# zeyadmohamedabdo/Visual-Question-Answering-VQA-system

Measured on AMD Instinct MI355X. Metric: image-question pairs/sec (train step), higher is better.
Workload: dtype bf16; 1 GPU; VQA train step fwd+CE+bwd+allreduce+clip+AdamW, batch 512/GPU, 3x224x224 images, 20 tokens, d=256, 4 text layers, 49 image tokens, 1000 answers, dropout on (BASELINE configs[2]); batch_per_gpu=512, global_batch=512, parallelism=dp1, reducer=off

## Files before the change

include/vqa_hip.h:

```cpp
#ifndef VQA_HIP_H
#define VQA_HIP_H
#include <stdint.h>
#ifdef __cplusplus
extern "C" {
#endif
typedef struct ihipStream_t* hipStream_t;

int vqa_igemm_mtiles(int M, int N, int loader);
int vqa_igemm_variant(int dtype, int loader, int M, int N, int Kw, int B, int H, int W, int C, int Ho, int Wo,
                      int R, int S, int stride, int pad);
int vqa_igemm(int dtype, int loader, const void* a, const void* w, void* out, const float* bias, const void* addend,
              const void* addmask, const void* outmask , float* stats, int M, int N, int Kw, int B, int H, int W, int C, int Ho, int Wo,
              int R, int S, int stride, int pad, int transposed, int relu, float drop_p, unsigned long long drop_seed,
              int stats_mode ,
              hipStream_t stream);
int vqa_linear_dgrad_act(int dtype, const void* dz, const void* wt, void* dx, const void* addend, const void* outact, float drop_p,
                         int M, int Kin, int N, hipStream_t stream);
int vqa_wgrad_plan(int dtype, int loader, int M, int N, int Kw, int B, int H, int W, int C, int R, int S, long long* ws_floats,
                   int* kind, int* tile_n, int* tile_k, int* nsplit);
int vqa_wgrad(int dtype, int loader, const void* dy, const void* x, float* dw, int M, int N, int Kw, int B, int H, int W,
              int C, int Ho, int Wo, int R, int S, int stride, int pad, float* ws, long long ws_floats, hipStream_t stream);
int vqa_pack_rows(int dtype, const float* in, void* out, int N, int K, int Kp, hipStream_t stream);
int vqa_pack_transpose(int dtype, const float* in, void* out, int N, int T, int C, int ldo, int col0, int flip, hipStream_t stream);
int vqa_pack_transpose_batch(int dtype, const float* flat, void* out, const long long* desc, int nd, int total_blocks, hipStream_t stream);
int vqa_fold_bn_batch(int dtype, const float* flat, void* wout, float* bout, const long long* desc, int nd, int total_blocks, float eps, hipStream_t stream);
int vqa_mx_quant(int dtype, const void* in, uint8_t* q, uint8_t* s, int M, int C, hipStream_t stream);
int vqa_fold_bn_mxfp8(const float* flat, uint8_t* wq, uint8_t* ws, float* bout, const long long* desc, int nd, int total_blocks, float eps,
                      hipStream_t stream);
int vqa_conv_mxfp8(const uint8_t* a, const uint8_t* as, const uint8_t* w, const uint8_t* ws, const float* bias, const void* addend,
                   void* out, uint8_t* oq, uint8_t* os, int M, int N, int B, int H, int W, int C, int Ho, int Wo, int R, int S,
                   int stride, int pad, int relu, hipStream_t stream);
int vqa_conv3x3_c64p_blocks(int B, int H, int W);
int vqa_conv3x3_c64p_bnred(const void* x, const void* w, void* out, const void* bn_y, const float* bn_coef, unsigned long long* bn_facc,
                           int B, int H, int W, hipStream_t stream);
int vqa_conv3x3_c64p_epi(const void* x, const void* w, void* out, const void* addend, const void* addmask, const void* outmask,
                         int B, int H, int W, hipStream_t stream);
int vqa_conv3x3_c64p(const void* x, const void* w, void* out, float* stats, int B, int H, int W,
                     int stats_mode , hipStream_t stream);
int vqa_gemm8p(const void* A, const void* B, void* C, int M, int N, int K, hipStream_t stream);
int vqa_gemm4w(const void* A, const void* B, void* C, int M, int N, int K, hipStream_t stream);
int vqa_conv8p_ok(int B, int H, int W, int C, int N);
int vqa_conv8p(const void* x, const void* w, void* out, unsigned long long* stats,
               const void* addend, const void* addmask, const void* outmask ,
               const void* bn_y, const float* bn_coef, unsigned long long* bn_facc ,
               int bn_selfmask ,
               const void* bn_y2, const float* bn_coef2 ,
               int B, int H, int W, int C, int N, int transposed, int stride , hipStream_t stream);
int vqa_conv3x3_c64p_bn(const void* y, const unsigned long long* acc, const float* gamma, const float* beta, float* running_mean,
                        float* running_var, long long* num_batches_tracked, float* coef_out, const void* w, void* out, float* stats,
                        int B, int H, int W, int stats_mode, double count, float momentum, float eps, hipStream_t stream);
int vqa_wgrad3x3_c64_bn_ok(int B, int H, int W);
int vqa_wgrad3x3_c64_bn(const void* y, const float* coef, const void* dy, float* dw , int B, int H, int W,
                        float* ws , long long ws_floats, hipStream_t stream);
int vqa_wgrad3x3_c128_blocks(int B, int H, int W);
int vqa_wgrad3x3_c128(const void* x, const void* dy, float* dw, int B, int H, int W, float* ws, long long ws_floats, hipStream_t stream);
int vqa_wgrad3x3_c64_blocks(int B, int H, int W);
int vqa_wgrad3x3_c64(const void* x, const void* dy, float* dw , int B, int H, int W,
                     float* ws ,
                     long long ws_floats, hipStream_t stream);
long long vqa_wgrad_group_ws(int dtype, int njobs, const int* M, const int* N, const int* Kw);
int vqa_wgrad_group(int dtype, int njobs, const void* const* dy, const void* const* x, float* const* dw, const int* M, const int* N,
                    const int* Kw, float* ws, long long ws_floats, hipStream_t stream);
int vqa_slab_reduce(const float* ws, float* dw, int nslabs, long long n, hipStream_t stream);
int vqa_dgrad_s2(int dtype, const void* dy, const void* dyd, const void* wt, void* out, int B, int H, int W, int C,
                 int Ho, int Wo, int N, int R, int pad, hipStream_t stream);
int vqa_stem_conv_blocks(int B, int H, int W);
int vqa_stem_pack(const float* w_krsc, void* wstem, hipStream_t stream);
int vqa_stem_conv(const float* img, const void* wstem, void* out, float* stats, int B, int H, int W, hipStream_t stream);
int vqa_stem_conv_pool_ok(int B, int H, int W);
int vqa_stem_conv_pool(const float* img, const void* wstem, const float* coef, void* out, int B, int H, int W, hipStream_t stream);
int vqa_stem_wgrad_blocks(int B, int H, int W);
int vqa_stem_wgrad(const float* img, const void* dy, float* dw , int B, int H, int W,
                   float* ws , long long ws_floats, hipStream_t stream);
int vqa_stem_wgrad_fused(const float* img, const void* y, const void* dpool, const uint8_t* idx, const float* coef,
                         const float* bcoef, float* dw, int B, int H, int W, float* ws, long long ws_floats, hipStream_t stream);
int vqa_stem_dgrad_pack(int dtype, const float* w_krsc, void* wpk, hipStream_t stream);
int vqa_stem_dgrad(int dtype, const void* dy, const void* wpk, float* dimg, int B, int H, int W, hipStream_t stream);
int vqa_stem_dgrad_fused_ok(int B, int H, int W);
int vqa_stem_dgrad_fused(const void* y, const void* dpool, const uint8_t* idx, const float* coef, const float* bcoef, const void* wpk,
                         float* dimg, int B, int H, int W, hipStream_t stream);

int vqa_bn_stats_finalize(const float* part, int tiles, int C, double count, const float* gamma, const float* beta,
                          float* running_mean, float* running_var, long long* num_batches_tracked, float momentum, float eps,
                          double* scratch , float* coef, hipStream_t stream);
int vqa_bn_eval_coef(int C, const float* gamma, const float* beta, const float* running_mean, const float* running_var,
                     float eps, float* coef, hipStream_t stream);
int vqa_bn_apply(int dtype, const void* y, const float* coef, const void* res, const float* rcoef, void* out,
                 long long numel, int C, int relu, hipStream_t stream);
int vqa_bn_apply_pool_chunks(int dtype, int HW, int C);
int vqa_bn_apply_pool(int dtype, const void* y, const float* coef, const void* res, const float* rcoef, void* out, int B, int HW, int C,
                      int relu, float* part, hipStream_t stream);
int vqa_bn_acc_words(int K, int C);
int vqa_bn_apply_acc(int dtype, const void* y, const unsigned long long* acc, const float* gamma, const float* beta, float* running_mean,
                     float* running_var, long long* num_batches_tracked, float* coef_out, const void* res,
                     const unsigned long long* racc, const float* rgamma, const float* rbeta, float* rrunning_mean, float* rrunning_var,
                     long long* rnum_batches_tracked, float* rcoef_out, void* out, int B, int HW, int C, int relu, double count,
                     float momentum, float eps, float* pool_part, hipStream_t stream);
int vqa_bn_bwd_blocks(long long rows);
int vqa_bn_bwd_reduce(int dtype, const void* dout, const void* outact, const void* y, const float* coef, const void* y2,
                      const float* coef2, float* slab , long long rows,
                      int C, int self_mask , int acc_mode, hipStream_t stream);
int vqa_bn_bwd_apply_acc(int dtype, const void* dout, const void* outact, const void* y, const unsigned long long* facc, const float* gamma,
                         const float* coef, float* dgamma, float* dbeta, void* dy, const void* y2, const float* gamma2, const float* coef2,
                         float* dgamma2, float* dbeta2, void* dy2, long long numel, int C, double count, int self_mask, hipStream_t stream);
int vqa_bn_bwd_finalize(const float* slab, int nblk, int C, int which, double count, const float* gamma, const float* coef,
                        int training, float* dgamma, float* dbeta, float* bcoef , hipStream_t stream);
int vqa_bn_bwd_apply(int dtype, const void* dout, const void* outact, const void* y, const float* bcoef, void* dy,
                     const void* y2, const float* bcoef2, void* dy2, long long numel, int C, const float* mask_coef ,
                     hipStream_t stream);

int vqa_stem_pool_fwd(int dtype, const void* y, const float* coef, void* out, uint8_t* idx, int B, int H, int W, int C, hipStream_t stream);
int vqa_stem_bwd_apply(int dtype, const void* dpool, const uint8_t* idx, const void* y, const float* coef, const float* bcoef,
                       void* dy, int B, int H, int W, int C, hipStream_t stream);

int vqa_se_fwd(int dtype, const void* x, const float* w1, const float* w2, float* pooled, float* hidden, float* scale,
               void* out, int B, int HW, int C, int Cr,
               const float* pool_part , int pool_chunks , hipStream_t stream);
int vqa_se_bwd_blocks(int dtype, int B, int HW, int C);
// ... 123 lines not shown
```

visual-question-answering-vqa-system_amd/_lib.py:

```python
from __future__ import annotations

import ctypes as C
import os

import torch

_HERE = os.path.dirname(os.path.abspath(__file__))
LIB_PATH = os.path.join(_HERE, "libvqa_hip.so")

P, I, F, D, LL, ULL = C.c_void_p, C.c_int, C.c_float, C.c_double, C.c_longlong, C.c_ulonglong

SIGNATURES = {
    "vqa_gemm8p": [P, P, P, I, I, I, P],
    "vqa_gemm4w": [P, P, P, I, I, I, P],
    "vqa_conv8p_ok": [I, I, I, I, I],
    "vqa_conv8p": [P, P, P, P, P, P, P, P, P, P, I, P, P, I, I, I, I, I, I, I, P],
    "vqa_igemm_mtiles": [I, I, I],
    "vqa_igemm_variant": [I] * 15,
    "vqa_igemm": [I, I, P, P, P, P, P, P, P, P] + [I] * 15 + [F, ULL, I, P],
    "vqa_linear_dgrad_act": [I, P, P, P, P, P, F, I, I, I, P],
    "vqa_wgrad_plan": [I] * 11 + [P, P, P, P, P],
    "vqa_wgrad": [I, I, P, P, P] + [I] * 13 + [P, LL, P],
    "vqa_pack_rows": [I, P, P, I, I, I, P],
    "vqa_pack_transpose": [I, P, P, I, I, I, I, I, I, P],
    "vqa_pack_transpose_batch": [I, P, P, P, I, I, P],
    "vqa_fold_bn_batch": [I, P, P, P, P, I, I, F, P],
    "vqa_mx_quant": [I, P, P, P, I, I, P],
    "vqa_fold_bn_mxfp8": [P, P, P, P, P, I, I, F, P],
    "vqa_conv_mxfp8": [P] * 9 + [I] * 13 + [P],
    "vqa_conv3x3_c64p_blocks": [I, I, I],
    "vqa_conv3x3_c64p": [P, P, P, P, I, I, I, I, P],
    "vqa_conv3x3_c64p_epi": [P, P, P, P, P, P, I, I, I, P],
    "vqa_conv3x3_c64p_bnred": [P, P, P, P, P, P, I, I, I, P],
    "vqa_conv3x3_c64p_bn": [P, P, P, P, P, P, P, P, P, P, P, I, I, I, I, D, F, F, P],
    "vqa_wgrad3x3_c64_bn_ok": [I, I, I],
    "vqa_wgrad3x3_c64_bn": [P, P, P, P, I, I, I, P, LL, P],
    "vqa_wgrad3x3_c128_blocks": [I, I, I],
    "vqa_wgrad3x3_c128": [P, P, P, I, I, I, P, LL, P],
    "vqa_wgrad3x3_c64_blocks": [I, I, I],
    "vqa_wgrad3x3_c64": [P, P, P, I, I, I, P, LL, P],
    "vqa_wgrad_group_ws": [I, I, P, P, P],
    "vqa_wgrad_group": [I, I, P, P, P, P, P, P, P, LL, P],
    "vqa_slab_reduce": [P, P, I, LL, P],
    "vqa_dgrad_s2": [I, P, P, P, P, I, I, I, I, I, I, I, I, I, P],
    "vqa_stem_conv_blocks": [I, I, I],
    "vqa_stem_pack": [P, P, P],
    "vqa_stem_conv": [P, P, P, P, I, I, I, P],
    "vqa_stem_conv_pool_ok": [I, I, I],
    "vqa_stem_conv_pool": [P, P, P, P, I, I, I, P],
    "vqa_stem_wgrad_blocks": [I, I, I],
    "vqa_stem_wgrad": [P, P, P, I, I, I, P, LL, P],
    "vqa_stem_wgrad_fused": [P, P, P, P, P, P, P, I, I, I, P, LL, P],
    "vqa_stem_dgrad_pack": [I, P, P, P],
    "vqa_stem_dgrad": [I, P, P, P, I, I, I, P],
    "vqa_stem_dgrad_fused_ok": [I, I, I],
    "vqa_stem_dgrad_fused": [P, P, P, P, P, P, P, I, I, I, P],
    "vqa_bn_stats_finalize": [P, I, I, D, P, P, P, P, P, F, F, P, P, P],
    "vqa_bn_eval_coef": [I, P, P, P, P, F, P, P],
    "vqa_bn_apply": [I, P, P, P, P, P, LL, I, I, P],
    "vqa_bn_apply_pool_chunks": [I, I, I],
    "vqa_bn_apply_pool": [I, P, P, P, P, P, I, I, I, I, P, P],
    "vqa_se_bwd_blocks": [I, I, I, I],
    "vqa_se_bwd_scratch": [I, I, I, I, I],
    "vqa_bn_bwd_blocks": [LL],
    "vqa_bn_bwd_reduce": [I, P, P, P, P, P, P, P, LL, I, I, I, P],
    "vqa_bn_acc_words": [I, I],
    "vqa_bn_apply_acc": [I, P, P, P, P, P, P, P, P, P, P, P, P, P, P, P, P, P, I, I, I, I, D, F, F, P, P],
    "vqa_bn_bwd_apply_acc": [I, P, P, P, P, P, P, P, P, P, P, P, P, P, P, P, LL, I, D, I, P],
    "vqa_bn_bwd_finalize": [P, I, I, I, D, P, P, I, P, P, P, P],
    "vqa_bn_bwd_apply": [I, P, P, P, P, P, P, P, P, LL, I, P, P],
    "vqa_stem_pool_fwd": [I, P, P, P, P, I, I, I, I, P],
    "vqa_stem_bwd_apply": [I, P, P, P, P, P, P, I, I, I, I, P],
    "vqa_se_fwd": [I, P, P, P, P, P, P, P, I, I, I, I, P, I, P],
    "vqa_se_bwd": [I, P, P, P, P, P, P, P, P, P, P, P, I, I, I, I, I, P, P, P, I, P],
    "vqa_spatial_fwd": [I, P, P, P, P, P, P, I, I, I, I, P],
    "vqa_spatial_bwd_scratch": [I, I, I],
    "vqa_spatial_bwd": [I, P, P, P, P, P, P, P, P, P, I, I, I, I, P],
    "vqa_nhwc_to_nchw": [I, P, P, I, I, I, P],
    "vqa_nchw_to_nhwc": [I, P, P, I, I, I, P],
    "vqa_embed_fwd": [I, P, P, P, P, I, I, I, I, F, F, ULL, P],
    "vqa_embed_bwd": [I, P, P, P, I, I, I, F, F, ULL, P],
    "vqa_layernorm_fwd": [I, P, P, P, P, P, I, I, F, F, ULL, P, I, P],
    "vqa_layernorm_bwd_ws": [I, I, I, I],
    "vqa_layernorm_bwd": [I, P, P, P, P, P, P, P, P, I, I, F, ULL, P, I, P, I, P],
    "vqa_layernorm_bwd_folds": [I, I, I, I, P],
    "vqa_attention_fwd": [I, P, P, P, I, I, I, P, P, P, I, I, I, I, I, I, F, ULL, P],
    "vqa_attention_fwd_mfma": [P, P, P, I, I, I, P, P, P, I, I, I, I, I, I, F, ULL, P],
    "vqa_attention_fwd_idx": [I, P, P, P, I, I, I, P, I, P, P, P, I, I, I, I, I, I, P],
    "vqa_attention_fwd_mfma_idx": [P, P, P, I, I, I, P, I, P, P, P, I, I, I, I, I, I, P],
    "vqa_attention_bwd": [I, P, I, P, P, P, I, I, I, P, P, P, P, I, I, I, I, I, I, I, I, F, ULL, P],
    "vqa_accuracy_update": [P, P, P, I, I, P],
    "vqa_attention_bwd_mfma": [P, I, P, P, P, I, I, I, P, P, P, P, I, I, I, I, I, I, I, I, F, ULL, P],
    "vqa_attention_bwd_dp": [I, P, I, P, P, P, I, I, I, P, P, P, P, P, I, I, I, I, I, I, I, I, F, ULL, P],
    "vqa_attention_bwd_mfma_dp": [P, I, P, P, P, I, I, I, P, P, P, P, P, I, I, I, I, I, I, I, I, F, ULL, P],
    "vqa_index_csr": [P, I, I, P, P, P],
    "vqa_attention_fwd_idx_train": [I, P, P, P, I, I, I, P, I, P, P, P, I, I, I, I, I, I, F, ULL, P],
    "vqa_attention_fwd_mfma_idx_train": [P, P, P, I, I, I, P, I, P, P, P, I, I, I, I, I, I, F, ULL, P],
    "vqa_attention_bwd_idx": [I, P, I, P, P, P, I, I, I, P, P, P, I, P, P, P, I, I, I, I, I, I, I, I, F, ULL, P],
    "vqa_attention_bwd_mfma_idx": [P, I, P, P, P, I, I, I, P, P, P, I, P, P, P, I, I, I, I, I, I, I, I, F, ULL, P],
    "vqa_masked_pool_fwd": [I, P, P, P, I, I, I, I, I, P],
    "vqa_masked_pool_bwd": [I, P, I, I, P, P, P, I, I, I, P],
    "vqa_masked_pool_pair_fwd": [I, P, P, P, P, I, I, I, P],
    "vqa_masked_pool_pair_bwd": [I, P, P, P, P, I, I, I, P],
    "vqa_gate_fwd": [I, P, P, P, I, I, P],
    "vqa_gate_bwd": [I, P, P, P, P, P, I, I, P],
    "vqa_add": [I, P, P, P, LL, P],
    "vqa_grad_tap_add": [I, P, P, I, I, I, I, P],
    "vqa_bias_act_bwd_ws": [I, I, I],
    "vqa_bias_act_bwd": [I, P, P, P, P, I, I, F, ULL, P, I, P],
    "vqa_bias_act_bwd_fold_rows": [I, I, I],
    "vqa_fold_group": [I, P, P, P, P, P, P, P, P],
    "vqa_cross_entropy": [I, P, P, P, P, P, I, I, F, P, P, P],
    "vqa_answer_scores": [P, P, P, P, I, I, I, I, P, P],
    "vqa_cross_entropy_soft": [I, P, P, P, I, P, P, P, I, I, F, P, P, P, P, P],
    "vqa_challenge_accuracy_update": [P, P, P, I, P, I, I, P],
    "vqa_convert": [I, I, P, P, LL, P],
    "vqa_sumsq": [P, LL, P, P],
    "vqa_image_normalize": [P, P, P, I, I, I, F, F, F, F, F, F, P],
    "vqa_image_color_jitter": [P, P, P, I, I, I, P, P, F, F, F, F, F, F, P, P],
    "vqa_image_resize_ws": [I, P, P, I, I, I],
    "vqa_image_resize": [P, P, P, P, P, I, I, I, I, I, P, P, P, F, F, F, F, F, F, P, LL, P],
    "vqa_pack_tokens": [P, P, P, P, I, I, I, I, I, I, P],
    "vqa_adamw": [P, P, P, P, LL, F, F, F, F, F, LL, P, F, F, P, P, P, P],
    "vqa_sumsq_ranges": [P, P, I, LL, P, P],
    "vqa_adamw_ranges": [P, P, P, P, P, I, LL, F, F, F, F, F, LL, P, F, F, P, P, P, P, I, P, P],
}
_RET_LL = {"vqa_image_resize_ws", "vqa_wgrad_group_ws", "vqa_spatial_bwd_scratch", "vqa_se_bwd_scratch", "vqa_layernorm_bwd_ws", "vqa_bias_act_bwd_ws"}
_NO_STATUS = _RET_LL | {"vqa_wgrad3x3_c64_blocks", "vqa_bn_acc_words", "vqa_bn_apply_pool_chunks", "vqa_se_bwd_blocks", "vqa_wgrad3x3_c128_blocks", "vqa_layernorm_bwd_folds", "vqa_bias_act_bwd_fold_rows", "vqa_conv3x3_c64p_blocks", "vqa_stem_wgrad_blocks", "vqa_igemm_mtiles", "vqa_igemm_variant", "vqa_bn_bwd_blocks", "vqa_stem_conv_blocks", "vqa_stem_conv_pool_ok", "vqa_stem_dgrad_fused_ok", "vqa_wgrad3x3_c64_bn_ok", "vqa_conv8p_ok"}

_lib = None


def lib() -> C.CDLL:
    global _lib
    if _lib is None:
        if not os.path.exists(LIB_PATH):
            raise RuntimeError(f"{LIB_PATH} is missing: build it with __graft_entry__.build() "
                               "(hipcc --offload-arch=gfx950); there is no CPU fallback")
        L = C.CDLL(LIB_PATH)
        for name, args in SIGNATURES.items():
            fn = getattr(L, name)
            fn.argtypes = args
            fn.restype = LL if name in _RET_LL else I
        _lib = L
    return _lib


def ptr(t):
    return None if t is None else t.data_ptr()


def stream() -> int:
    return torch.cuda.current_stream().cuda_stream


_HOOK = [None]


def call(name: str, *args):
    fn = getattr(lib(), name)
    hook = _HOOK[0]
    done = hook(name, args) if hook is not None else None
    rc = fn(*args, stream())
    if done is not None:
        done()
    if rc != 0:
        raise RuntimeError(f"{name} failed with status {rc}" + (" (argument/shape error)" if rc == 1000 else " (hipError_t)"))


def count(name: str, *args) -> int:
    assert name in _NO_STATUS
    return getattr(lib(), name)(*args)


def dt(t_or_dtype) -> int:
    d = t_or_dtype.dtype if isinstance(t_or_dtype, torch.Tensor) else t_or_dtype
    if d == torch.float32:
        return 0
    if d == torch.bfloat16:
        return 1
    raise TypeError(f"unsupported dtype {d}")
# ... 1 lines not shown
```

visual-question-answering-vqa-system_amd/build.py:

```python
import os
import subprocess
import sys

HERE = os.path.dirname(os.path.abspath(__file__))
CSRC = os.path.join(HERE, "csrc")
SOURCES = ["gemm_conv.hip", "cnn_ops.hip", "token_ops.hip", "stem_conv.hip", "conv_c64.hip", "input_ops.hip", "gemm8p.hip", "mxfp8.hip", "stem_dgrad.hip"]
LIB = os.path.join(HERE, "libvqa_hip.so")
HIPCC = os.environ.get("HIPCC", "/opt/rocm/bin/hipcc")
FLAGS = ["--offload-arch=gfx950", "-O3", "-std=c++17", "-fPIC", "-Wno-unused-result"]


def _stale():
    if not os.path.exists(LIB):
        return True
    t = os.path.getmtime(LIB)
    import glob
    deps = [os.path.join(CSRC, f) for f in SOURCES] + glob.glob(os.path.join(CSRC, "*.h"))
    return any(os.path.getmtime(d) > t for d in deps)


def build_lib(force=False, verbose=True):
    if not force and not _stale():
        return LIB
    objs = []
    procs = []
    for src in SOURCES:
        obj = os.path.join(CSRC, src.replace(".hip", ".o"))
        objs.append(obj)
        cmd = [HIPCC] + FLAGS + ["-c", os.path.join(CSRC, src), "-o", obj]
        if verbose:
            print(" ".join(cmd), flush=True)
        procs.append((cmd, subprocess.Popen(cmd)))
    for cmd, p in procs:
        if p.wait() != 0:
            raise RuntimeError("hipcc failed: " + " ".join(cmd))
    cmd = [HIPCC, "--offload-arch=gfx950", "-shared", "-fPIC", "-o", LIB] + objs
    if verbose:
        print(" ".join(cmd), flush=True)
    subprocess.check_call(cmd)
    return LIB


if __name__ == "__main__":
    build_lib(force="--force" in sys.argv)
    print(LIB)
```

visual-question-answering-vqa-system_amd/engine.py:

```python
from __future__ import annotations

import math
from typing import Callable, Dict, List, Optional

import torch

from . import kernels as K
from . import layout as LY
from ._lib import call, dt, ptr


def _streams_overlap(a: "torch.cuda.Stream", b: "torch.cuda.Stream", cycles: int = 1_500_000) -> bool:
    ea, eb = torch.cuda.Event(), torch.cuda.Event()
    with torch.cuda.stream(a):
        torch.cuda._sleep(cycles)
        ea.record()
    with torch.cuda.stream(b):
        torch.cuda._sleep(1000)
        eb.record()
    eb.synchronize()
    ok = not ea.query()
    ea.synchronize()
    return ok

# ... 1 lines not shown
def pick_concurrent_streams(device, n: int, avoid=(), tries: int = 12):
    main = torch.cuda.current_stream(device)
    if torch.cuda.is_current_stream_capturing():
        return tuple(torch.cuda.Stream(device=device) for _ in range(n))
    chosen, spare = [], []
    for _ in range(tries):
        if len(chosen) == n:
            break
        c = torch.cuda.Stream(device=device)
        if all(_streams_overlap(o, c) for o in [main, *avoid, *chosen]):
            chosen.append(c)
        else:
            spare.append(c)
    while len(chosen) < n:
        chosen.append(spare.pop(0) if spare else torch.cuda.Stream(device=device))
    return tuple(chosen)


class HipEngine:
    def __init__(self, cfg: dict, entries: List[LY.Entry], flat: torch.Tensor, buffers: Dict[str, torch.Tensor],
                 compute_dtype: torch.dtype):
        self.cfg = cfg
        self.entries = entries
        self.E = {e.name: e for e in entries}
        self.flat = flat
        self.buf = buffers
        self.dtype = compute_dtype
        self.seed_base = 0x5EED
        self.seed_rank = None
        self.step_id = 0
        self.wsrc = flat
        self._wsrc_fresh = False
        self._wt: Dict[str, torch.Tensor] = {}
        self._wt_plan: Dict[str, tuple] = {}
        self._wt_table = None
        self._wt_buf = None
        self._deferred = []
        self._keep = []
        self._wgq = []
        self._foldq = []
        self._foldq2 = []
        self._plan = None
        self._bwd_G = None
        self.fuse_act_dgrad = True
        self.fuse_se_pool = True
        self.fuse_se_bnred = True
        self.fuse_bn_finalize = True
        self.fuse_bn_conv = True
        self.use_conv8p = True
        self.conv8p_n_multiple = 128
        self.conv8p_bwd_n_multiple = 128
        self.pack_off_main = True
        self.hoist_cross = True
        self.use_c64p_epi = True
        self.fuse_bn1_reduce = True
        self.use_conv8p_bwd = True
        self._accbuf = None
        self._accpos = 0
        self._stem_fcoef = None
        self.fold_eval = True
        self._fold = None
        self.infer_precision = "bf16"
        self._foldmx = None
        self.stem_w = None
        self.side, self.side2 = pick_concurrent_streams(flat.device, 2) if flat.is_cuda else (None, None)
        self.two_streams = True
        self.capture = None
        self.capture_io = None
        self.fuse_stem_eval = True
        self.mark = None

    def P(self, name):
        e = self.E[name]
        return self.flat[e.offset: e.offset + e.numel]

    def Wm(self, name):
        return LY.mat_of(self.wsrc, self.E[name])

    def _packT(self, key, pieces, rows, ld):
        t = self._wt.get(key)
        if t is None:
            t = torch.empty((rows, ld), device=self.flat.device, dtype=self.dtype)
            for off, n, tt, c, col0, flip in pieces:
                K.pack_transpose(self.flat[off: off + n * tt * c].view(n, tt, c), self.dtype, out=t, ldo=ld, col0=col0, flip=flip)
            self._wt[key] = t
            self._wt_plan[key] = (tuple(pieces), rows, ld)
            self._wt_table = None
        return t

    def Wt(self, name):
        e = self.E[name]
        n, c = e.shape[0], e.shape[1]
        tt = e.numel // (n * c)
        return self._packT(name, [(e.offset, n, tt, c, 0, False)], c, tt * n)

    def _pack_planned(self):
        if not self._wt_plan:
            return
        if self._wt_table is None or self._wt_table[0].device != self.flat.device:
            rowsd, views, dst, blk = [], [], 0, 0
            for key, (pieces, rows, ld) in self._wt_plan.items():
                for off, n, tt, c, col0, flip in pieces:
                    rowsd.append([off, dst, n, tt, c, ld, col0, int(flip), blk, 0])
                    blk += tt * ((n + 31) // 32) * ((c + 31) // 32)
                views.append((key, dst, rows, ld))
                dst += (rows * ld + 7) // 8 * 8
# ... 1347 lines not shown
                            y2=rec.get("yd"), coef2=rec.get("cd"),
                            gamma2=self.P(p + ".downsample.1.weight") if has_ds else None,
                            dgamma2=gs(p + ".downsample.1.weight") if has_ds else None,
                            dbeta2=gs(p + ".downsample.1.bias") if has_ds else None,
                            slab=pre[0] if (pre and not pre_acc) else None, nb=pre[1] if (pre and not pre_acc) else 0,
                            facc=(pre[0] if pre_acc else (self._acc(K.L.count("vqa_bn_acc_words", 3, Cout)) if bacc else None)), facc_filled=pre_acc)
        g2 = rec["g2"]; B, Ho, Wo = g2[0], g2[1], g2[2]
        if not tw2:
            pass
        elif rec["a1"] is None:
            self._off_path([dy2], lambda: K.wgrad3x3_c64_bn(rec["y1"], rec["c1"], dy2, LY.mat_of(G, self.E[p + ".conv2.weight"]), B, Ho, Wo), defer=last)
        elif self._c64w_ok(B, Ho, Wo, Cout, Cout, 3, 1):
            self._off_path([dy2], lambda: K.wgrad3x3_c64(rec["a1"], dy2, LY.mat_of(G, self.E[p + ".conv2.weight"]), B, Ho, Wo), defer=last)
        elif self._c128w_ok(B, Ho, Wo, Cout, Cout, 1):
            self._off_path([dy2], lambda: K.wgrad3x3_c128(rec["a1"], dy2, LY.mat_of(G, self.E[p + ".conv2.weight"]), B, Ho, Wo))
        else:
            self._off_path([dy2], lambda: K.wgrad(dy2, rec["a1"], LY.mat_of(G, self.E[p + ".conv2.weight"]), M, Cout, 9 * Cout, g2, dtype=T))
        facc1 = None
        if self._c64p_ok(B, Ho, Wo, Cout, Cout, 3, 1) and bacc and self.fuse_bn1_reduce:
            facc1 = self._acc(K.L.count("vqa_bn_acc_words", 3, Cout))
            da1 = K.conv3x3_c64p_bnred(dy2, self._wflip(p + ".conv2.weight"), B, Ho, Wo, rec["y1"], rec["c1"], facc1)
        elif self._c64p_ok(B, Ho, Wo, Cout, Cout, 3, 1):
            da1, _, _ = K.conv3x3_c64p(dy2, self._wflip(p + ".conv2.weight"), B, Ho, Wo)
        elif self.use_conv8p_bwd and self._c8p_ok(B, Ho, Wo, Cout, Cout, 3, 1, 1, bwd=True):
            if bacc and self.fuse_bn1_reduce:
                facc1 = self._acc(K.L.count("vqa_bn_acc_words", 3, Cout))
            da1 = K.conv8p(dy2, self.Wt(p + ".conv2.weight"), B, Ho, Wo, Cout, Cout, transposed=1,
                           bnred=(rec["y1"], rec["c1"], facc1) if facc1 is not None else None)
        else:
            geom_d2 = (B, Ho, Wo, Cout, Ho, Wo, 3, 3, 1, 1)
            da1, _, _ = K.igemm(dy2, self.Wt(p + ".conv2.weight"), M, Cout, 9 * Cout, geom_d2, dtype=T, transposed=1)
        dy1, _ = K.bn_bwd(da1, None, rec["y1"], rec["c1"], self.P(p + ".bn1.weight"), Cout, training,
                          gs(p + ".bn1.weight"), gs(p + ".bn1.bias"), self_mask=True,
                          facc=facc1 if facc1 is not None else (self._acc(K.L.count("vqa_bn_acc_words", 3, Cout)) if bacc else None),
                          facc_filled=facc1 is not None)
        g1 = rec["g1"]; H, W, stride = g1[1], g1[2], g1[8]
        if not tw1:
            pass
        elif self._c64w_ok(B, H, W, Cin, Cout, 3, stride):
            self._off_path([dy1], lambda: K.wgrad3x3_c64(rec["x"], dy1, LY.mat_of(G, self.E[p + ".conv1.weight"]), B, H, W), defer=last)
        elif self._c128w_ok(B, H, W, Cin, Cout, stride):
            self._off_path([dy1], lambda: K.wgrad3x3_c128(rec["x"], dy1, LY.mat_of(G, self.E[p + ".conv1.weight"]), B, H, W))
        else:
            self._off_path([dy1], lambda: K.wgrad(dy1, rec["x"], LY.mat_of(G, self.E[p + ".conv1.weight"]), M, Cout, 9 * Cin, g1, dtype=T))
        Md = B * H * W
        geom_d1 = (B, Ho, Wo, Cout, H, W, 3, 3, stride, 1)
        if has_ds:
            gd = rec["gd"]
            if twd:
                self._off_path([dyd], lambda: K.wgrad(dyd, rec["x"], LY.mat_of(G, self.E[p + ".downsample.0.weight"]), M, Cout, Cin, gd, dtype=T))
            if stride == 2 and H % 2 == 0 and W % 2 == 0:
                wt = self._packT(p + ".dgrad2", [(self.E[p + ".conv1.weight"].offset, Cout, 9, Cin, 0, False),
                                                 (self.E[p + ".downsample.0.weight"].offset, Cout, 1, Cin, 9 * Cout, False)], Cin, 10 * Cout)
                dx = K.dgrad_s2(dy1, dyd, wt, B, Ho, Wo, Cout, H, W, Cin, 3, 1, dtype=T)
            else:
                geom_dd = (B, Ho, Wo, Cout, H, W, 1, 1, stride, 0)
                dxd, _, _ = K.igemm(dyd, self.Wt(p + ".downsample.0.weight"), Md, Cin, Cout, geom_dd, dtype=T, transposed=1)
                dx, _, _ = K.igemm(dy1, self.Wt(p + ".conv1.weight"), Md, Cin, 9 * Cout, geom_d1, dtype=T, transposed=1, addend=dxd)
        elif self.use_c64p_epi and self._c64p_ok(B, H, W, Cout, Cin, 3, stride):
            dx = K.conv3x3_c64p_epi(dy1, self._wflip(p + ".conv1.weight"), B, H, W, addend=dout, addmask=out_act, outmask=outmask)
        elif self.use_conv8p_bwd and stride == 1 and self._c8p_ok(B, H, W, Cout, Cin, 3, stride, 1, bwd=True):
            dx = K.conv8p(dy1, self.Wt(p + ".conv1.weight"), B, H, W, Cout, Cin, transposed=1, addend=dout, addmask=out_act, outmask=outmask)
        else:
            dx, _, _ = K.igemm(dy1, self.Wt(p + ".conv1.weight"), Md, Cin, 9 * Cout, geom_d1, dtype=T, transposed=1,
                               addend=dout, addmask=out_act, outmask=outmask)
        if self.capture is not None:
            self.capture[p] = dict(dout=dout, masked=masked, handed=hand is not None, dy2=dy2, dyd=dyd, da1=da1, dy1=dy1, dx=dx)
        return dx
```

visual-question-answering-vqa-system_amd/kernels.py:

```python
from __future__ import annotations

import os

import torch

from . import _lib as L
from ._lib import call, dt, ptr

LOADER_NHWC, LOADER_STEM = 0, 1

PROFILE = None
PROFILE_VARIANTS = []
PROFILE_STAGED = {}


def prof_begin():
    if PROFILE is None:
        return None
    e0 = torch.cuda.Event(enable_timing=True)
    e0.record()
    return e0


def prof_end(e0, sym, flops, nbytes):
# ... 178 lines not shown
    call("vqa_conv8p", ptr(x), ptr(w), ptr(out), ptr(stats_acc), ptr(addend), ptr(addmask), ptr(outmask), ptr(bn_y), ptr(bn_coef), ptr(bn_facc),
         int(bool(bn_self)), ptr(bn_y2), ptr(bn_coef2),
         B, H, W, C, N, int(transposed), int(stride))
    if e0 is not None:
        sym = "conv8p_kernel<2, 4>" if N % 256 == 0 else "conv8p_kernel<4, 2>"
        flops = 2.0 * out.shape[0] * N * 9 * C
        e1 = prof_end(e0, sym, flops,
                      (B * H * W * C + out.shape[0] * N * (1 + sum(t is not None for t in (addend, addmask, outmask, bn_y, bn_y2))) + N * 9 * C) * 2)
        PROFILE_VARIANTS.append((sym, "with epilogue inputs" if (addend is not None or outmask is not None or bnred is not None) else "plain",
                                 flops, e0, e1))
        bmp, bn = (224, 256) if N % 256 == 0 else (448, 128)
        rpt = bmp * 7 // 8 if out.shape[0] % (bmp * 7 // 8) == 0 else bmp
        PROFILE_STAGED[sym] = PROFILE_STAGED.get(sym, 0) + (-(-out.shape[0] // rpt)) * (N // bn) * (9 * C // 64) * (bmp + bn) * 128
    return out


def c64w_blocks(B, H, W) -> int:
    return L.count("vqa_wgrad3x3_c64_blocks", B, H, W)


def wgrad3x3_c64(x, dy, dw, B, H, W):
    e0 = prof_begin()
    wsf = c64w_blocks(B, H, W) * 64 * 576
    ws = torch.empty(wsf, device=x.device, dtype=torch.float32)
    call("vqa_wgrad3x3_c64", ptr(x), ptr(dy), ptr(dw), B, H, W, ptr(ws), wsf)
    if e0 is not None:
        prof_end(e0, "wgrad3x3_c64", 2.0 * B * H * W * 64 * 576, 2 * B * H * W * 64 * 2)


def c128_wgrad_blocks(B, H, W):
    return L.count("vqa_wgrad3x3_c128_blocks", B, H, W)


def wgrad3x3_c128(x, dy, dw, B, H, W):
    e0 = prof_begin()
    wsf = c128_wgrad_blocks(B, H, W) * 128 * 576
    ws = torch.empty(wsf, device=x.device, dtype=torch.float32)
    call("vqa_wgrad3x3_c128", ptr(x), ptr(dy), ptr(dw), B, H, W, ptr(ws), wsf)
    if e0 is not None:
        prof_end(e0, "wgrad3x3_c128p_kernel", 2.0 * B * H * W * 128 * 1152, 2 * B * H * W * 128 * 2)


def dgrad_s2(dy, dyd, wt, B, H, W, C, Ho, Wo, N, R, pad, *, dtype):
    out = torch.empty((B * Ho * Wo, N), device=dy.device, dtype=dtype)
    e0 = prof_begin()
    call("vqa_dgrad_s2", dt(dtype), ptr(dy), ptr(dyd), ptr(wt), ptr(out), B, H, W, C, Ho, Wo, N, R, pad)
    if e0 is not None:
        flops = 2.0 * B * H * W * C * N * (R * R + (1 if dyd is not None else 0))
        prof_end(e0, f"igemm_kernel<{_tname(dtype)}, 128, {64 if N <= 64 else 128}, 2, 4, {_bk(dtype)}, 2, 2, 0>", flops,
                 (B * H * W * C * (2 if dyd is not None else 1) + B * Ho * Wo * N) * 2)
    return out


def stem_wgrad(img, dy, dw, B, H, W):
    Ho, Wo = (H + 6 - 7) // 2 + 1, (W + 6 - 7) // 2 + 1
    e0 = prof_begin()
    ws, wsf = stem_wgrad_scratch(img.device, B, H, W)
    call("vqa_stem_wgrad", ptr(img), ptr(dy), ptr(dw), B, H, W, ptr(ws), wsf)
    if e0 is not None:
        prof_end(e0, "stem_wgrad_kernel<false>", 2.0 * B * Ho * Wo * 64 * 147, B * 3 * H * W * 4 + B * Ho * Wo * 64 * 2)


def stem_wgrad_scratch(device, B, H, W):
    wsf = L.count("vqa_stem_wgrad_blocks", B, H, W) * 64 * 147
    return torch.empty(wsf, device=device, dtype=torch.float32), wsf


def stem_dgrad_pack(w_krsc, dtype):
    wpk = torch.empty(16 * 1024, device=w_krsc.device, dtype=dtype)
    call("vqa_stem_dgrad_pack", dt(dtype), ptr(w_krsc), ptr(wpk))
    return wpk


def stem_dgrad_fused_ok(B, H, W) -> bool:
    return L.count("vqa_stem_dgrad_fused_ok", B, H, W) > 0


def _stem_dgrad_cost(B, H, W):
    Ho, Wo = (H + 6 - 7) // 2 + 1, (W + 6 - 7) // 2 + 1
    return Ho, Wo, 2.0 * B * Ho * Wo * 64 * 147


def stem_dgrad(dy, wpk, B, H, W):
    dimg = torch.empty((B, 3, H, W), device=dy.device, dtype=torch.float32)
    Ho, Wo, flops = _stem_dgrad_cost(B, H, W)
    e0 = prof_begin()
    call("vqa_stem_dgrad", dt(dy), ptr(dy), ptr(wpk), ptr(dimg), B, H, W)
    if e0 is not None:
        prof_end(e0, f"stem_dgrad_kernel<{'bf16' if dy.dtype == torch.bfloat16 else 'f32'},false>", flops,
                 dy.numel() * dy.element_size() + dimg.numel() * 4)
    return dimg


def stem_dgrad_fused(y, dpool, idx, coef, bc, wpk, B, H, W):
    dimg = torch.empty((B, 3, H, W), device=y.device, dtype=torch.float32)
    Ho, Wo, flops = _stem_dgrad_cost(B, H, W)
    e0 = prof_begin()
    call("vqa_stem_dgrad_fused", ptr(y), ptr(dpool), ptr(idx), ptr(coef), ptr(bc), ptr(wpk), ptr(dimg), B, H, W)
    if e0 is not None:
        prof_end(e0, "stem_dgrad_kernel<bf16,true>", flops, B * Ho * Wo * 64 * 2 + dpool.numel() * 3 + dimg.numel() * 4)
    return dimg


def stem_conv_blocks(B, H, W) -> int:
    return L.count("vqa_stem_conv_blocks", B, H, W)

# ... 287 lines not shown
```

Measured before the change: 41060 pairs/s.

## Add persistent phase-decomposed stride-2 dgrad kernel with LDS DMA pipelining

Adds a specialised bf16 kernel for the stride-2 3x3 conv backward-data path (C=128 to N=64) that decomposes the transposed convolution into four output parity classes. It stages dy patches and weight taps in LDS through buffer_load-to-LDS DMA with triple-buffered weights and double-buffered activations, and runs as a persistent grid over row blocks. The kernel replaces the generic igemm-based dgrad_s2 for the downsampling block in ResNet backward. This skips the zero-stuffed work of the generic kernel and overlaps loads with MFMA, at the cost of hand-tuned waitcnt logic that is fragile.

```diff
diff --git a/include/vqa_hip.h b/include/vqa_hip.h
--- a/include/vqa_hip.h
+++ b/include/vqa_hip.h
@@ -64,6 +64,8 @@
 int vqa_slab_reduce(const float* ws, float* dw, int nslabs, long long n, hipStream_t stream);
 int vqa_dgrad_s2(int dtype, const void* dy, const void* dyd, const void* wt, void* out, int B, int H, int W, int C,
                  int Ho, int Wo, int N, int R, int pad, hipStream_t stream);
+int vqa_dgrad_s2p_ok(int B, int H, int W, int C, int N);
+int vqa_dgrad_s2p(const void* dy, const void* dyd, const void* wt, void* out, int B, int H, int W, int C, int N, hipStream_t stream);
 int vqa_stem_conv_blocks(int B, int H, int W);
 int vqa_stem_pack(const float* w_krsc, void* wstem, hipStream_t stream);
 int vqa_stem_conv(const float* img, const void* wstem, void* out, float* stats, int B, int H, int W, hipStream_t stream);
diff --git a/visual-question-answering-vqa-system_amd/_lib.py b/visual-question-answering-vqa-system_amd/_lib.py
--- a/visual-question-answering-vqa-system_amd/_lib.py
+++ b/visual-question-answering-vqa-system_amd/_lib.py
@@ -43,6 +43,8 @@
     "vqa_wgrad_group": [I, I, P, P, P, P, P, P, P, LL, P],
     "vqa_slab_reduce": [P, P, I, LL, P],
     "vqa_dgrad_s2": [I, P, P, P, P, I, I, I, I, I, I, I, I, I, P],
+    "vqa_dgrad_s2p_ok": [I, I, I, I, I],
+    "vqa_dgrad_s2p": [P, P, P, P, I, I, I, I, I, P],
     "vqa_stem_conv_blocks": [I, I, I],
     "vqa_stem_pack": [P, P, P],
     "vqa_stem_conv": [P, P, P, P, I, I, I, P],
@@ -126,7 +128,7 @@
     "vqa_adamw_ranges": [P, P, P, P, P, I, LL, F, F, F, F, F, LL, P, F, F, P, P, P, P, I, P, P],
 }
 _RET_LL = {"vqa_image_resize_ws", "vqa_wgrad_group_ws", "vqa_spatial_bwd_scratch", "vqa_se_bwd_scratch", "vqa_layernorm_bwd_ws", "vqa_bias_act_bwd_ws"}
-_NO_STATUS = _RET_LL | {"vqa_wgrad3x3_c64_blocks", "vqa_bn_acc_words", "vqa_bn_apply_pool_chunks", "vqa_se_bwd_blocks", "vqa_wgrad3x3_c128_blocks", "vqa_layernorm_bwd_folds", "vqa_bias_act_bwd_fold_rows", "vqa_conv3x3_c64p_blocks", "vqa_stem_wgrad_blocks", "vqa_igemm_mtiles", "vqa_igemm_variant", "vqa_bn_bwd_blocks", "vqa_stem_conv_blocks", "vqa_stem_conv_pool_ok", "vqa_stem_dgrad_fused_ok", "vqa_wgrad3x3_c64_bn_ok", "vqa_conv8p_ok"}
+_NO_STATUS = _RET_LL | {"vqa_wgrad3x3_c64_blocks", "vqa_bn_acc_words", "vqa_bn_apply_pool_chunks", "vqa_se_bwd_blocks", "vqa_wgrad3x3_c128_blocks", "vqa_layernorm_bwd_folds", "vqa_bias_act_bwd_fold_rows", "vqa_conv3x3_c64p_blocks", "vqa_stem_wgrad_blocks", "vqa_igemm_mtiles", "vqa_igemm_variant", "vqa_bn_bwd_blocks", "vqa_stem_conv_blocks", "vqa_stem_conv_pool_ok", "vqa_stem_dgrad_fused_ok", "vqa_wgrad3x3_c64_bn_ok", "vqa_conv8p_ok", "vqa_dgrad_s2p_ok"}
 
 _lib = None
 
diff --git a/visual-question-answering-vqa-system_amd/build.py b/visual-question-answering-vqa-system_amd/build.py
--- a/visual-question-answering-vqa-system_amd/build.py
+++ b/visual-question-answering-vqa-system_amd/build.py
@@ -4,7 +4,7 @@
 
 HERE = os.path.dirname(os.path.abspath(__file__))
 CSRC = os.path.join(HERE, "csrc")
-SOURCES = ["gemm_conv.hip", "cnn_ops.hip", "token_ops.hip", "stem_conv.hip", "conv_c64.hip", "input_ops.hip", "gemm8p.hip", "mxfp8.hip", "stem_dgrad.hip"]
+SOURCES = ["gemm_conv.hip", "cnn_ops.hip", "token_ops.hip", "stem_conv.hip", "conv_c64.hip", "input_ops.hip", "gemm8p.hip", "mxfp8.hip", "stem_dgrad.hip", "dgrad_s2p.hip"]
 LIB = os.path.join(HERE, "libvqa_hip.so")
 HIPCC = os.environ.get("HIPCC", "/opt/rocm/bin/hipcc")
 FLAGS = ["--offload-arch=gfx950", "-O3", "-std=c++17", "-fPIC", "-Wno-unused-result"]
diff --git a/visual-question-answering-vqa-system_amd/csrc/dgrad_s2p.hip b/visual-question-answering-vqa-system_amd/csrc/dgrad_s2p.hip
--- /dev/null
+++ b/visual-question-answering-vqa-system_amd/csrc/dgrad_s2p.hip
@@ -0,0 +1,216 @@
+#include <utility>
+#include "common.h"
+
+namespace {
+constexpr int S2P_C = 128, S2P_N = 64, S2P_ROWB = S2P_C * 2;
+constexpr int S2P_WTILE = S2P_N * S2P_ROWB, S2P_NWBUF = 3, S2P_JUNK = 1024;
+constexpr int S2P_OOB = (int)0x80000000;
+typedef int i32x4_s2p __attribute__((ext_vector_type(4)));
+
+__device__ __forceinline__ void dma16_s2p(i32x4_s2p rs, unsigned lds_addr, int voff) {
+  lds_addr = __builtin_amdgcn_readfirstlane(lds_addr);
+  asm volatile("s_mov_b32 m0, %2\n\ts_nop 0\n\tbuffer_load_dwordx4 %0, %1, 0 offen lds" ::"v"(voff), "s"(rs), "s"(lds_addr) : "memory");
+}
+__device__ __forceinline__ i32x4_s2p rsrc_s2p(const void* ptr, unsigned bytes) {
+  const unsigned long long a = (unsigned long long)ptr;
+  return i32x4_s2p{(int)(unsigned)a, (int)((unsigned)(a >> 32) & 0xffffu), (int)bytes, 0x00020000};
+}
+template <class F, int... I>
+__device__ __forceinline__ void static_for_s2p(F&& f, std::integer_sequence<int, I...>) { (f(std::integral_constant<int, I>{}), ...); }
+}
+
+struct DgradS2pParams {
+  const bf16_t* dy; const bf16_t* dyd; const bf16_t* wt; bf16_t* out;
+  int B, H, W, RB, rblocks, nblocks, Ktot;
+  unsigned dy_bytes, wt_bytes;
+  int patch_bytes, dyd_bytes;
+};
+
+__global__ __launch_bounds__(512, 2) void dgrad_s2p_kernel(DgradS2pParams p) {
+  extern __shared__ __attribute__((aligned(16))) char smem[];
+  const int tid = threadIdx.x, lane = tid & 63, g = lane >> 4, li = lane & 15;
+  const int wave = __builtin_amdgcn_readfirstlane(tid >> 6);
+  const int wn = wave & 1, wm = wave >> 1;
+  const int W = p.W, H = p.H, PW = W + 1;
+  const int npatch = (p.RB + 1) * PW, npp = (npatch + 3) >> 2;
+  const unsigned lds0 = (unsigned)(size_t)((__attribute__((address_space(3))) char*)smem);
+  const unsigned dbase = (unsigned)(2 * p.patch_bytes), wbase = dbase + (unsigned)p.dyd_bytes, junk = wbase + S2P_NWBUF * S2P_WTILE;
+  const i32x4_s2p rsY = rsrc_s2p(p.dy, p.dy_bytes), rsD = rsrc_s2p(p.dyd, p.dyd ? p.dy_bytes : 0u), rsW = rsrc_s2p(p.wt, p.wt_bytes);
+  const int first = p.dyd ? 0 : 1;
+  const int dpx = lane >> 4, dj = lane & 15;
+
+  auto issue_w = [&](int st, int slot) {
+    const int tap = st == 0 ? 9 : st - 1;
+#pragma unroll
+    for (int i = 0; i < 2; ++i) {
+      const int piece = wave * 2 + i, n = piece * 4 + dpx, f = (n & 3) | (((n >> 3) & 3) << 2);
+      if (st >= 0) dma16_s2p(rsW, lds0 + wbase + (unsigned)(slot * S2P_WTILE + piece * 1024), (n * p.Ktot + tap * S2P_C) * 2 + ((dj ^ f) << 4));
+      else dma16_s2p(rsW, lds0 + junk, S2P_OOB);
+    }
+  };
+  auto issue_res = [&](int blk, int buf, int id) {
+    const int b = blk / p.rblocks, ih0 = (blk - b * p.rblocks) * p.RB;
+    const int rows = H - ih0 < p.RB ? H - ih0 : p.RB, npx = rows * W;
+    if (blk < p.nblocks && id < npp) {
+      const int lin = id * 4 + dpx, prow = lin / PW, pcol = lin - prow * PW, ih = ih0 + prow;
+      const bool ok = lin < npatch && pcol < W && ih < H;
+      dma16_s2p(rsY, lds0 + (unsigned)(buf * p.patch_bytes + id * 1024),
+                ok ? ((b * H + ih) * W + pcol) * S2P_ROWB + ((dj ^ (lin & 15)) << 4) : S2P_OOB);
+    } else if (blk < p.nblocks && p.dyd && (id - npp) * 4 < npx) {
+      const int px = (id - npp) * 4 + dpx;
+      dma16_s2p(rsD, lds0 + dbase + (unsigned)((id - npp) * 1024),
+                px < npx ? ((b * H + ih0) * W + px) * S2P_ROWB + ((dj ^ (px & 15)) << 4) : S2P_OOB);
+    } else dma16_s2p(rsY, lds0 + junk, S2P_OOB);
+  };
+  const int nres = npp + (p.dyd ? (p.RB * W + 3) >> 2 : 0);
+  const int cap = (9 - first) * 8;
+
+  unsigned wa[2];
+#pragma unroll
+  for (int nt = 0; nt < 2; ++nt) {
+    const int n = wn * 32 + 8 * (li >> 2) + 4 * nt + (li & 3);
+    wa[nt] = (unsigned)(n * S2P_ROWB + ((g ^ li) << 4));
+  }
+
+  int blk = blockIdx.x, buf = 0, slot = 0, kprev = -1;
+  for (int id = wave; id < nres; id += 8) issue_res(blk, 0, id);
+  issue_w(first, 0); issue_w(first + 1, 1);
+  asm volatile("s_waitcnt vmcnt(0)" ::: "memory");
+  __builtin_amdgcn_s_barrier();
+
+  for (; blk < p.nblocks; blk += gridDim.x, buf ^= 1) {
+    const int nxt = blk + gridDim.x;
+    const int b = blk / p.rblocks, ih0 = (blk - b * p.rblocks) * p.RB;
+    const int rows = H - ih0 < p.RB ? H - ih0 : p.RB, npx = rows * W, mtiles = (npx + 15) >> 4;
+    unsigned pa[2][4], da[2];
+    int orow[2], ocol[2]; bool live[2];
+#pragma unroll
+    for (int mi = 0; mi < 2; ++mi) {
+      const int px = (wm + 4 * mi) * 16 + li;
+      live[mi] = px < npx;
+      const int pxc = live[mi] ? px : 0;
+      orow[mi] = pxc / W; ocol[mi] = pxc - orow[mi] * W;
+#pragma unroll
+      for (int sh = 0; sh < 4; ++sh) {
+        const int lin = (orow[mi] + (sh >> 1)) * PW + ocol[mi] + (sh & 1);
+        pa[mi][sh] = (unsigned)(buf * p.patch_bytes + lin * S2P_ROWB + ((g ^ (lin & 15)) << 4));
+      }
+      da[mi] = dbase + (unsigned)(pxc * S2P_ROWB + ((g ^ (pxc & 15)) << 4));
+    }
+    const bool has0 = wm < mtiles, has1 = wm + 4 < mtiles;
+
+    f32x4 acc[4][2][2];
+#pragma unroll
+    for (int c = 0; c < 4; ++c)
+#pragma unroll
+      for (int mi = 0; mi < 2; ++mi)
+#pragma unroll
+        for (int nt = 0; nt < 2; ++nt) acc[c][mi][nt] = f32x4{0.f, 0.f, 0.f, 0.f};
+
+    static_for_s2p([&](auto E_) {
+      constexpr int E = decltype(E_)::value, T = E == 0 ? 9 : E - 1;
+      constexpr int r = T < 9 ? T / 3 : 1, s_ = T < 9 ? T % 3 : 1;
+      constexpr int ph = (r + 1) & 1, pw = (s_ + 1) & 1, cls = ph * 2 + pw;
+      constexpr int sh = ((ph + 1 - r) / 2) * 2 + (pw + 1 - s_) / 2;
+      if (E >= first) {
+        if (E == first) {
+          if (kprev == 8) asm volatile("s_waitcnt vmcnt(11)" ::: "memory");
+          else if (kprev == 4) asm volatile("s_waitcnt vmcnt(7)" ::: "memory");
+          else if (kprev >= 0) asm volatile("s_waitcnt vmcnt(3)" ::: "memory");
+          if (kprev >= 0) __builtin_amdgcn_s_barrier();
+        } else {
+          asm volatile("s_waitcnt vmcnt(3)" ::: "memory");
+          __builtin_amdgcn_s_barrier();
+        }
+        {
+          const int id = (E - first) * 8 + wave;
+          const bool take = E < 9 && !(E == 0 && id >= npp);
+          issue_res(take ? nxt : p.nblocks, buf ^ 1, id);
+        }
+        {
+          const int st = E + 2 <= 9 ? E + 2 : first + E + 2 - 10;
+          issue_w(E + 2 <= 9 || nxt < p.nblocks ? st : -1, slot >= 1 ? slot - 1 : 2);
+        }
+        const char* wt = smem + wbase + slot * S2P_WTILE;
+#pragma unroll
+        for (int ks = 0; ks < S2P_C / 32; ++ks) {
+          const bf16x8 a0 = *reinterpret_cast<const bf16x8*>(wt + (wa[0] ^ (unsigned)(ks << 6)));
+          const bf16x8 a1 = *reinterpret_cast<const bf16x8*>(wt + (wa[1] ^ (unsigned)(ks << 6)));
+#pragma unroll
+          for (int mi = 0; mi < 2; ++mi) {
+            const bf16x8 x = *reinterpret_cast<const bf16x8*>(smem + ((T < 9 ? pa[mi][sh] : da[mi]) ^ (unsigned)(ks << 6)));
+            acc[cls][mi][0] = __builtin_amdgcn_mfma_f32_16x16x32_bf16(a0, x, acc[cls][mi][0], 0, 0, 0);
+            acc[cls][mi][1] = __builtin_amdgcn_mfma_f32_16x16x32_bf16(a1, x, acc[cls][mi][1], 0, 0, 0);
+          }
+        }
+        slot = slot == 2 ? 0 : slot + 1;
+      }
+    }, std::make_integer_sequence<int, 10>{});
+
+    typedef __attribute__((ext_vector_type(2))) float f32x2_t;
+    typedef __attribute__((ext_vector_type(2))) __bf16 bf16x2_t;
+#pragma unroll
+    for (int mi = 0; mi < 2; ++mi) {
+      if (!(mi ? has1 : has0)) continue;
+#pragma unroll
+      for (int c = 0; c < 4; ++c) {
+        u32x4 o;
+#pragma unroll
+        for (int nt = 0; nt < 2; ++nt) {
+          o[2 * nt] = __builtin_bit_cast(uint32_t, __builtin_convertvector((f32x2_t){acc[c][mi][nt][0], acc[c][mi][nt][1]}, bf16x2_t));
+          o[2 * nt + 1] = __builtin_bit_cast(uint32_t, __builtin_convertvector((f32x2_t){acc[c][mi][nt][2], acc[c][mi][nt][3]}, bf16x2_t));
+        }
+        const size_t oh = (size_t)2 * (ih0 + orow[mi]) + (c >> 1), ow = (size_t)2 * ocol[mi] + (c & 1);
+        if (live[mi]) *reinterpret_cast<u32x4*>(p.out + (((size_t)b * 2 * H + oh) * 2 * W + ow) * S2P_N + wn * 32 + 8 * g) = o;
+      }
+    }
+    kprev = 4 * ((has0 ? 1 : 0) + (has1 ? 1 : 0));
+    if (nxt < p.nblocks && (nres > cap || npp < 8)) {
+      for (int id = wave; id < nres; id += 8)
+        if (id >= cap || (id < 8 && id >= npp)) issue_res(nxt, buf ^ 1, id);
+      asm volatile("s_waitcnt vmcnt(0)" ::: "memory");
+    }
+  }
+  asm volatile("s_waitcnt vmcnt(0)" ::: "memory");
+}
+
+namespace {
+bool s2p_plan(int B, int H, int W, int C, int N, int* RB, int* patch_bytes, int* dyd_bytes) {
+  if (B <= 0 || H <= 0 || W <= 0 || W > 128 || C != S2P_C || N != S2P_N) return false;
+  if ((unsigned long long)B * H * W * S2P_ROWB >= 0x7fffffffull) return false;
+  int rb = 128 / W; if (rb > H) rb = H;
+  const int nb = (H + rb - 1) / rb;
+  rb = (H + nb - 1) / nb;
+  for (; rb >= 1; --rb) {
+    *RB = rb;
+    *patch_bytes = ((rb + 1) * (W + 1) + 3) / 4 * 1024;
+    *dyd_bytes = (rb * W + 3) / 4 * 1024;
+    if (2 * *patch_bytes + *dyd_bytes + S2P_NWBUF * S2P_WTILE + S2P_JUNK <= 160 * 1024) return true;
+  }
+  return false;
+}
+}
+
+extern "C" {
+
+int vqa_dgrad_s2p_ok(int B, int H, int W, int C, int N) {
+  int rb, pb, db;
+  return s2p_plan(B, H, W, C, N, &rb, &pb, &db) ? 1 : 0;
+}
+
+int vqa_dgrad_s2p(const void* dy, const void* dyd, const void* wt, void* out, int B, int H, int W, int C, int N, hipStream_t st) {
+  DgradS2pParams p;
+  if (!dy || !wt || !out || !s2p_plan(B, H, W, C, N, &p.RB, &p.patch_bytes, &p.dyd_bytes)) return VQA_EARG;
+  p.dy = (const bf16_t*)dy; p.dyd = (const bf16_t*)dyd; p.wt = (const bf16_t*)wt; p.out = (bf16_t*)out;
+  p.B = B; p.H = H; p.W = W; p.rblocks = (H + p.RB - 1) / p.RB; p.nblocks = B * p.rblocks; p.Ktot = 9 * C + (dyd ? C : 0);
+  p.dy_bytes = (unsigned)((size_t)B * H * W * S2P_ROWB); p.wt_bytes = (unsigned)((size_t)N * p.Ktot * 2);
+  const int smem = 2 * p.patch_bytes + p.dyd_bytes + S2P_NWBUF * S2P_WTILE + S2P_JUNK;
+  int dev = 0, cus = 0;
+  if (hipGetDevice(&dev) != hipSuccess || hipDeviceGetAttribute(&cus, hipDeviceAttributeMultiprocessorCount, dev) != hipSuccess || cus <= 0) cus = 256;
+  (void)vqa_ensure_lds(reinterpret_cast<const void*>(&dgrad_s2p_kernel), smem);
+  hipLaunchKernelGGL(dgrad_s2p_kernel, dim3(p.nblocks < cus ? p.nblocks : cus), dim3(512), smem, st, p);
+  VQA_LAUNCH_CHECK();
+  return VQA_OK;
+}
+
+}
diff --git a/visual-question-answering-vqa-system_amd/engine.py b/visual-question-answering-vqa-system_amd/engine.py
--- a/visual-question-answering-vqa-system_amd/engine.py
+++ b/visual-question-answering-vqa-system_amd/engine.py
@@ -77,6 +77,7 @@
         self.conv8p_bwd_n_multiple = 128
         self.pack_off_main = True
         self.hoist_cross = True
+        self.use_dgrad_s2p = True
         self.use_c64p_epi = True
         self.fuse_bn1_reduce = True
         self.use_conv8p_bwd = True
@@ -1530,7 +1531,10 @@
             if stride == 2 and H % 2 == 0 and W % 2 == 0:
                 wt = self._packT(p + ".dgrad2", [(self.E[p + ".conv1.weight"].offset, Cout, 9, Cin, 0, False),
                                                  (self.E[p + ".downsample.0.weight"].offset, Cout, 1, Cin, 9 * Cout, False)], Cin, 10 * Cout)
-                dx = K.dgrad_s2(dy1, dyd, wt, B, Ho, Wo, Cout, H, W, Cin, 3, 1, dtype=T)
+                if self.use_dgrad_s2p and T == torch.bfloat16 and K.dgrad_s2p_ok(B, Ho, Wo, Cout, Cin):
+                    dx = K.dgrad_s2p(dy1, dyd, wt, B, Ho, Wo, Cout, Cin)
+                else:
+                    dx = K.dgrad_s2(dy1, dyd, wt, B, Ho, Wo, Cout, H, W, Cin, 3, 1, dtype=T)
             else:
                 geom_dd = (B, Ho, Wo, Cout, H, W, 1, 1, stride, 0)
                 dxd, _, _ = K.igemm(dyd, self.Wt(p + ".downsample.0.weight"), Md, Cin, Cout, geom_dd, dtype=T, transposed=1)
diff --git a/visual-question-answering-vqa-system_amd/kernels.py b/visual-question-answering-vqa-system_amd/kernels.py
--- a/visual-question-answering-vqa-system_amd/kernels.py
+++ b/visual-question-answering-vqa-system_amd/kernels.py
@@ -254,6 +254,20 @@
     return out
 
 
+def dgrad_s2p_ok(B, H, W, C, N) -> bool:
+    return bool(L.count("vqa_dgrad_s2p_ok", B, H, W, C, N))
+
+
+def dgrad_s2p(dy, dyd, wt, B, H, W, C, N):
+    out = torch.empty((B * 4 * H * W, N), device=dy.device, dtype=torch.bfloat16)
+    e0 = prof_begin()
+    call("vqa_dgrad_s2p", ptr(dy), ptr(dyd), ptr(wt), ptr(out), B, H, W, C, N)
+    if e0 is not None:
+        prof_end(e0, "dgrad_s2p_kernel", 2.0 * B * H * W * C * N * (9 + (1 if dyd is not None else 0)),
+                 (B * H * W * C * (2 if dyd is not None else 1) + B * 4 * H * W * N) * 2)
+    return out
+
+
 def stem_wgrad(img, dy, dw, B, H, W):
     Ho, Wo = (H + 6 - 7) // 2 + 1, (W + 6 - 7) // 2 + 1
     e0 = prof_begin()
```

Result: no change. 41160 pairs/s (median of 3 runs) (+0.2%).
